# ofsoundof/GRL-Image-Restoration

Hardware: AMD Instinct MI355X
Metric: LQ megapixels/s, GRL-Base x4 SR, 256x256 LQ tiles (higher is better)
Workload: dtype f16 MFMA operands (attention, linear, conv), f32 accumulate + residual stream; 1 GPU; BASELINE configs[2]: GRL-Base x4 SR, 256x256 LQ tiles, ckpt geometry (window 32, stripe 64x64, anchor /2), random-init weights with checkpoint-like logit scales exp(min(ln 100 + 0.3 N(0,1), ln 100)): about half of the heads at the clamp, the regime of every released checkpoint; logit_scale_regime=checkpoint-like, parallelism=tile-sharded x1, no data-path collective, precision_mode=fast

## Files before the change

### grl_image_restoration_amd/csrc/cab_conv2.hip

```cpp
#include "common.h"
#include "grl_hip_internal.h"
#include <stdlib.h>

namespace {

constexpr int C2_TH = 8, C2_TW = 32;
constexpr int C2_HH = C2_TH + 2, C2_HW = C2_TW + 2;
constexpr int C2_SEG = 7;
constexpr int C2_PXB = C2_SEG * 16;
constexpr int C2_NPIECE = C2_HH * C2_HW * C2_SEG;
constexpr int C2_WAVES = 8, C2_THREADS = C2_WAVES * 64;
constexpr int C2_ROUNDS = (C2_NPIECE + C2_THREADS - 1) / C2_THREADS;
constexpr int C2_HALO_B = C2_ROUNDS * C2_THREADS * 16;
constexpr int C2_KSTEPS = 14, C2_NG = 3;
constexpr int C2_KREAL = 9 * 48;

typedef __attribute__((__vector_size__(4 * sizeof(uint32_t)))) uint32_t c2_u32x4;

__global__ __launch_bounds__(C2_THREADS) void cab_conv2_kernel(GrlCabConv2Args p) {
    extern __shared__ __attribute__((aligned(1024))) char smem[];
    const int tid = threadIdx.x, lane = tid & 63, wave = tid >> 6;
    const int wave_u = __builtin_amdgcn_readfirstlane(wave);
    const int r16 = lane & 15, g4 = lane >> 4;
    const int cs = wave_u & 3, ph = wave_u >> 2;
    const int img = blockIdx.x / p.wgs_per_image, wgi = blockIdx.x % p.wgs_per_image;
    const int tiles_x = (p.W + C2_TW - 1) / C2_TW, tiles_y = (p.H + C2_TH - 1) / C2_TH, ntiles = tiles_x * tiles_y;
    const uint32_t lds0 = (uint32_t)(uintptr_t)(__attribute__((address_space(3))) void*)smem;

    gemm_x8 A[C2_NG][C2_KSTEPS];
    {
        const gemm_x8* src = (const gemm_x8*)p.blob + (int64_t)(3 * cs) * C2_KSTEPS * 64 + lane;
#pragma unroll
        for (int g = 0; g < C2_NG; ++g)
#pragma unroll
            for (int s = 0; s < C2_KSTEPS; ++s) A[g][s] = src[(g * C2_KSTEPS + s) * 64];
    }
    f32x4 pool[C2_NG];
#pragma unroll
    for (int g = 0; g < C2_NG; ++g) pool[g] = f32x4{0, 0, 0, 0};
    float* bias_s = (float*)(smem + 2 * C2_HALO_B);
    if (tid < 192) bias_s[tid] = p.bias[tid];
    __syncthreads();
    const float* bias_l = bias_s + 48 * cs + 4 * g4;
    const bool hi2 = g4 >= 2;

    int h0;
    {
        const int px = tid / C2_SEG, seg = tid - px * C2_SEG, hy = px / C2_HW, hx = px - hy * C2_HW;
        h0 = hy << 16 | hx << 4 | seg;
    }
    c2_u32x4 xsrd;
    {
        const uint64_t a = (uint64_t)((const gemm_t*)p.x + (int64_t)img * p.H * p.W * p.ldx);
        xsrd[0] = __builtin_amdgcn_readfirstlane((uint32_t)a);
        xsrd[1] = __builtin_amdgcn_readfirstlane((uint32_t)(a >> 32) & 0xffffu);
        xsrd[2] = (uint32_t)((int64_t)p.H * p.W * p.ldx * 2);
        xsrd[3] = 0x00020000u;
    }
    auto prefetch = [&](int tile, int buf) {
        const int ty = tile / tiles_x, tx = tile - ty * tiles_x;
        const int y0 = ty * C2_TH - 1, x0 = tx * C2_TW - 1;
        int hy = h0 >> 16, hx = (h0 >> 4) & 0xfff, seg = h0 & 15;
#pragma unroll 1
        for (int j = 0; j < C2_ROUNDS; ++j) {
            if (j > 0) {
                static_assert(C2_THREADS == 73 * C2_SEG + 1 && 73 == 2 * C2_HW + 5, "piece stepping");
                seg += 1; hx += 5; hy += 2;
                if (seg >= C2_SEG) { seg -= C2_SEG; hx += 1; }
                if (hx >= C2_HW) { hx -= C2_HW; hy += 1; }
            }
            const int gy = y0 + hy, gx = x0 + hx;
            const bool ok = hy < C2_HH && gy >= 0 && gy < p.H && gx >= 0 && gx < p.W;
            const uint32_t voff = ok ? (uint32_t)(((int64_t)gy * p.W + gx) * p.ldx * 2 + seg * 16) : 0xfffffff0u;
            const uint32_t m0v = __builtin_amdgcn_readfirstlane(lds0 + buf * C2_HALO_B + (j * C2_THREADS + wave_u * 64) * 16);
            asm volatile("s_mov_b32 m0, %0\n\ts_nop 4\n\tbuffer_load_dwordx4 %1, %2, 0 offen lds" ::"s"(m0v), "v"(voff), "s"(xsrd) : "memory");
        }
    };

    int tile = wgi;
    if (tile < ntiles) prefetch(tile, 0);
    for (int it = 0; tile < ntiles; ++it, tile += p.wgs_per_image) {
        asm volatile("s_waitcnt vmcnt(0)" ::: "memory");
        __builtin_amdgcn_s_barrier();
        if (tile + p.wgs_per_image < ntiles) prefetch(tile + p.wgs_per_image, (it + 1) & 1);
        const int ty = tile / tiles_x, tx = tile - ty * tiles_x;
        const char* hb = smem + (it & 1) * C2_HALO_B;
#pragma unroll 1
        for (int rr = 0; rr < 4; ++rr) {
            const int r = 4 * ph + rr;
            const int y = ty * C2_TH + r;
            const char* u0 = hb + (r * C2_HW + r16) * C2_PXB + 16 * g4;
            const char* uA = u0 + (hi2 ? C2_PXB - 96 : 0);
            const char* uB = u0 + (hi2 ? (C2_HW - 2) * C2_PXB - 96 : 0);
            const char* uC = u0 + (hi2 ? -32 : 0);
            f32x4 acc0[C2_NG], acc1[C2_NG];
#pragma unroll
            for (int g = 0; g < C2_NG; ++g) { acc0[g] = *(const f32x4*)(bias_l + 16 * g); acc1[g] = acc0[g]; }
#pragma unroll
            for (int s = 0; s < C2_KSTEPS; ++s) {
                constexpr int TAPOFF[9] = {0, C2_PXB, 2 * C2_PXB, C2_HW * C2_PXB, (C2_HW + 1) * C2_PXB, (C2_HW + 2) * C2_PXB,
// ... 75 lines not shown
```

### grl_image_restoration_amd/csrc/conv.hip

```cpp
#include "common.h"
#include "grl_hip_internal.h"
#include <stdlib.h>

namespace {

constexpr int TH = 8, TW = 32;
constexpr int CWAVES = 8;
constexpr int HALO_W = TW + 2, HALO_H = TH + 2;

template <int KC, int NT>
__global__ __launch_bounds__(CWAVES * 64) void conv3x3_kernel(GrlConvArgs p) {
    extern __shared__ __attribute__((aligned(16))) char smem[];
    constexpr int ROWB = KC * 2 + 16;
    constexpr int KS = KC / 32;
    constexpr int IN_BYTES = HALO_H * HALO_W * ROWB;
    constexpr int WT_BYTES = NT * 16 * ROWB;
    constexpr int SEG_ROW = KC / 8;
    constexpr int WSEGS = NT * 16 * SEG_ROW;
    constexpr int WPT = (WSEGS + CWAVES * 64 - 1) / (CWAVES * 64);
    char* in_s = smem;
    char* wt_s = smem + IN_BYTES;

    const int tid = threadIdx.x, lane = tid & 63, wave = tid >> 6;
    const int r16 = lane & 15, g4 = lane >> 4;
    const int x0 = blockIdx.x * TW, y0 = blockIdx.y * TH, b = blockIdx.z;
    const int nkc = p.CinP / KC;

    f32x4 acc[2][NT];
#pragma unroll
    for (int mt = 0; mt < 2; ++mt)
#pragma unroll
        for (int nt = 0; nt < NT; ++nt) acc[mt][nt] = f32x4{0, 0, 0, 0};

    gemm_x8 wpre[WPT];
    auto load_w = [&](int tap, int kc) {
        const gemm_t* src = (const gemm_t*)p.w + (int64_t)tap * p.w_tap_stride + kc * KC;
#pragma unroll
        for (int i = 0; i < WPT; ++i) {
            const int s = tid + i * CWAVES * 64;
            if (s < WSEGS) {
                const int rr = s / SEG_ROW, cc = s % SEG_ROW;
                wpre[i] = *(const gemm_x8*)(src + (int64_t)rr * p.CinP + cc * 8);
            }
        }
    };
    auto store_w = [&](int buf) {
#pragma unroll
        for (int i = 0; i < WPT; ++i) {
            const int s = tid + i * CWAVES * 64;
            if (s < WSEGS) {
                const int rr = s / SEG_ROW, cc = s % SEG_ROW;
                *(gemm_x8*)(wt_s + buf * WT_BYTES + rr * ROWB + cc * 16) = wpre[i];
            }
        }
    };

    const int csrc = p.x_split == 3 ? p.CinP / 3 : (p.x_split == 2 ? p.CinP / 2 : p.CinP);
    const float xsc = p.x_scale != 0.0f ? p.x_scale : 1.0f;
    const float osc = p.out_scale != 0.0f ? p.out_scale : 1.0f;
    auto stage_input = [&](int kc) {
#pragma unroll 2
        for (int s = tid; s < HALO_H * HALO_W * SEG_ROW; s += CWAVES * 64) {
            const int pix = s / SEG_ROW, cc = s % SEG_ROW;
            const int vch = kc * KC + cc * 8;
            int part = 0, ch0 = vch;
            if (p.x_split >= 2) {
                part = vch / csrc;
                ch0 = vch - part * csrc;
            }
            const int hy = pix / HALO_W, hx = pix % HALO_W;
            const int gy = y0 + hy - 1, gx = x0 + hx - 1;
            gemm_x8 v = {0, 0, 0, 0, 0, 0, 0, 0};
            if (gy >= 0 && gy < p.H && gx >= 0 && gx < p.W) {
                const int64_t row = ((int64_t)b * p.H + gy) * p.W + gx;
                if (p.x_dtype == GRL_DT_F16) {
                    v = *(const gemm_x8*)((const gemm_t*)p.x + row * p.ldx + ch0);
                } else {
                    const float4* q = (const float4*)((const float*)p.x + row * p.ldx + ch0);
                    float4 a0, a1;
                    if (p.x_cols > 0) {
                        a0 = ch0 < p.x_cols ? q[0] : float4{0, 0, 0, 0};
                        a1 = ch0 + 4 < p.x_cols ? q[1] : float4{0, 0, 0, 0};
                    } else {
                        a0 = q[0]; a1 = q[1];
                    }
                    const float e[8] = {a0.x * xsc, a0.y * xsc, a0.z * xsc, a0.w * xsc, a1.x * xsc, a1.y * xsc, a1.z * xsc, a1.w * xsc};
#pragma unroll
                    for (int i = 0; i < 8; ++i) v[i] = to_f16(e[i]);
                    if (p.x_split >= 2 && part == 1) {
#pragma unroll
                        for (int i = 0; i < 8; ++i) v[i] = (f16)(e[i] - (float)v[i]);
                    }
                }
            }
            *(gemm_x8*)(in_s + pix * ROWB + cc * 16) = v;
        }
    };
    auto mfma_tap = [&](int tap, const char* wb) {
        const int dy = tap / 3, dx = tap - dy * 3;
        gemm_x8 af[2][KS];
#pragma unroll
        for (int mt = 0; mt < 2; ++mt)
#pragma unroll
            for (int ks = 0; ks < KS; ++ks)
                af[mt][ks] = *(const gemm_x8*)(in_s + ((wave + dy) * HALO_W + (16 * mt + r16 + dx)) * ROWB + (32 * ks + 8 * g4) * 2);
#pragma unroll
        for (int ks = 0; ks < KS; ++ks) {
#pragma unroll
            for (int nt = 0; nt < NT; ++nt) {
                const gemm_x8 wf = *(const gemm_x8*)(wb + (nt * 16 + r16) * ROWB + (32 * ks + 8 * g4) * 2);
                acc[0][nt] = mfma16_gemm(wf, af[0][ks], acc[0][nt]);
                acc[1][nt] = mfma16_gemm(wf, af[1][ks], acc[1][nt]);
            }
        }
    };

    for (int kc = 0; kc < nkc; ++kc) {
        load_w(0, kc);
        __syncthreads();
        stage_input(kc);
        store_w(0);
        __syncthreads();
        for (int tap = 0; tap < 9; ++tap) {
            if (tap < 8) load_w(tap + 1, kc);
            mfma_tap(tap, wt_s + (tap & 1) * WT_BYTES);
            if (tap < 8) {
                store_w((tap + 1) & 1);
                __syncthreads();
            }
        }
    }

    const int gy = y0 + wave;
    float psum[NT][4];
#pragma unroll
    for (int nt = 0; nt < NT; ++nt)
#pragma unroll
        for (int e = 0; e < 4; ++e) psum[nt][e] = 0.f;

    const bool staged = p.out_dtype != GRL_DT_F32 && p.shuffle_r <= 1 && p.resid == nullptr;
    constexpr int ZSEGS = ((NT * 16 + 31) / 32 * 32 - NT * 16) / 8;
    constexpr int OROW = (NT * 2 + ZSEGS) * 16 + 16;
    if (staged) {
        __syncthreads();
#pragma unroll
        for (int mt = 0; mt < 2; ++mt) {
            const int gx = x0 + 16 * mt + r16;
            const bool valid = gy < p.H && gx < p.W;
            char* prow = smem + (wave * TW + 16 * mt + r16) * OROW;
#pragma unroll
            for (int nt = 0; nt < NT; ++nt) {
                const int c = 16 * nt + 4 * g4;
                const float4 b4 = *(const float4*)(p.bias + c);
                float v[4] = {fmaf(acc[mt][nt][0], osc, b4.x), fmaf(acc[mt][nt][1], osc, b4.y), fmaf(acc[mt][nt][2], osc, b4.z), fmaf(acc[mt][nt][3], osc, b4.w)};
                if (p.act == 1) {
{
                        const f32x2v ga = gelu_erf2(f32x2v{v[0], v[1]}), gb = gelu_erf2(f32x2v{v[2], v[3]});
                        v[0] = ga.x; v[1] = ga.y; v[2] = gb.x; v[3] = gb.y;
                    }
                } else if (p.act == 2) {
#pragma unroll
                    for (int e = 0; e < 4; ++e) v[e] = v[e] > 0.f ? v[e] : v[e] * p.slope;
                }
                if (valid) {
#pragma unroll
                    for (int e = 0; e < 4; ++e) psum[nt][e] += v[e];
                }
                uint2 pk;
                pk.x = pack_f16(v[0], v[1]);
                pk.y = pack_f16(v[2], v[3]);
                *(uint2*)(prow + c * 2) = pk;
            }
        }
        const int zs = (p.ldo >= (NT * 16 + 31) / 32 * 32) ? ZSEGS : 0;
        if (ZSEGS > 0 && tid < TH * TW) {
#pragma unroll
            for (int z = 0; z < ZSEGS; ++z) *(uint4*)(smem + tid * OROW + (NT * 2 + z) * 16) = uint4{0, 0, 0, 0};
        }
        __syncthreads();
        const int SEGS = NT * 2 + zs;
        for (int i = tid; i < TH * TW * SEGS; i += CWAVES * 64) {
            const int px = i / SEGS, sg = i - px * SEGS;
            const int ty = px / TW, tx = px - ty * TW;
            const int oy = y0 + ty, ox = x0 + tx;
            if (oy < p.H && ox < p.W) {
                const int64_t row = ((int64_t)b * p.H + oy) * p.W + ox;
                *(uint4*)((gemm_t*)p.out + row * p.ldo + sg * 8) = *(const uint4*)(smem + px * OROW + sg * 16);
            }
        }
    }
#pragma unroll
    for (int mt = 0; mt < (staged ? 0 : 2); ++mt) {
        const int gx = x0 + 16 * mt + r16;
        const bool valid = gy < p.H && gx < p.W;
        const int64_t row = ((int64_t)b * p.H + gy) * p.W + gx;
#pragma unroll
        for (int nt = 0; nt < NT; ++nt) {
            const int c = 16 * nt + 4 * g4;
            const float4 b4 = *(const float4*)(p.bias + c);
            float v[4] = {fmaf(acc[mt][nt][0], osc, b4.x), fmaf(acc[mt][nt][1], osc, b4.y), fmaf(acc[mt][nt][2], osc, b4.z), fmaf(acc[mt][nt][3], osc, b4.w)};
            if (p.act == 1) {
{
                    const f32x2v ga = gelu_erf2(f32x2v{v[0], v[1]}), gb = gelu_erf2(f32x2v{v[2], v[3]});
                    v[0] = ga.x; v[1] = ga.y; v[2] = gb.x; v[3] = gb.y;
                }
            } else if (p.act == 2) {
#pragma unroll
                for (int e = 0; e < 4; ++e) v[e] = v[e] > 0.f ? v[e] : v[e] * p.slope;
            }
            if (valid) {
                if (p.pool_partial != nullptr) {
#pragma unroll
                    for (int e = 0; e < 4; ++e) psum[nt][e] += v[e];
                }
                if (p.resid != nullptr) {
                    const float4 r4 = *(const float4*)(p.resid + row * p.ldr + c);
                    v[0] += r4.x; v[1] += r4.y; v[2] += r4.z; v[3] += r4.w;
                }
                int64_t orow = row;
                int oc = c;
                bool keep = true;
                if (p.shuffle_r > 1) {
                    const int r = p.shuffle_r, cg = p.shuffle_cg;
                    const int q = c / cg;
                    const int ij = p.shuffle_ij0 + q;
                    oc = c - q * cg;
                    keep = ij < r * r;
                    orow = ((int64_t)b * p.H * r + (gy * r + ij / r)) * (p.W * r) + (gx * r + ij % r);
                }
                if (!keep || (p.n_store > 0 && oc >= p.n_store)) {
                } else if (p.out_dtype != GRL_DT_F32) {
                    uint2 pk;
                    pk.x = pack_f16(v[0], v[1]);
                    pk.y = pack_f16(v[2], v[3]);
                    *(uint2*)((gemm_t*)p.out + orow * p.ldo + oc) = pk;
                } else {
                    *(float4*)((float*)p.out + orow * p.ldo + oc) = float4{v[0], v[1], v[2], v[3]};
                }
            }
        }
    }
    if (p.pool_partial != nullptr) {
        __syncthreads();
        float* red = (float*)smem;
#pragma unroll
        for (int nt = 0; nt < NT; ++nt)
#pragma unroll
            for (int e = 0; e < 4; ++e) {
                const float s = row16_sum(psum[nt][e]);
                if (r16 == 0) red[wave * (NT * 16) + 16 * nt + 4 * g4 + e] = s;
            }
        __syncthreads();
        const int wg = (blockIdx.z * gridDim.y + blockIdx.y) * gridDim.x + blockIdx.x;
        for (int c = tid; c < NT * 16; c += CWAVES * 64) {
            float s = 0.f;
#pragma unroll
            for (int w = 0; w < CWAVES; ++w) s += red[w * (NT * 16) + c];
            p.pool_partial[(int64_t)wg * p.pool_stride + c] = s;
        }
    }
}

template <int KC, int NT>
int launch_conv(const GrlConvArgs& p, hipStream_t st) {
    const dim3 grid((p.W + TW - 1) / TW, (p.H + TH - 1) / TH, p.B);
    const size_t rowb = KC * 2 + 16;
    const size_t lds_in = (size_t)HALO_H * HALO_W * rowb;
    size_t lds = lds_in + 2 * (size_t)NT * 16 * rowb;
    const size_t tile_b = (size_t)TH * TW * (NT * 32 + 32 + 16);
    if (lds < tile_b) lds = tile_b;
    auto kfn = conv3x3_kernel<KC, NT>;
    hipError_t e = hipFuncSetAttribute((const void*)kfn, hipFuncAttributeMaxDynamicSharedMemorySize, (int)lds);
    if (e != hipSuccess) return (int)e;
    hipLaunchKernelGGL(kfn, grid, dim3(CWAVES * 64), lds, st, p);
    GRL_CHECK_LAUNCH();
    return 0;
}

template <int KC>
int launch_conv_nt(const GrlConvArgs& p, hipStream_t st) {
    switch (p.CoutP / 16) {
        case 1: return launch_conv<KC, 1>(p, st);
        case 2: return launch_conv<KC, 2>(p, st);
        case 3: return launch_conv<KC, 3>(p, st);
        case 4: return launch_conv<KC, 4>(p, st);
        case 6: return launch_conv<KC, 6>(p, st);
        case 8: return launch_conv<KC, 8>(p, st);
        case 12: return launch_conv<KC, 12>(p, st);
        default: return GRL_ERR_UNSUPPORTED;
    }
}

__global__ __launch_bounds__(1024) void se_kernel(const float* __restrict__ partial, int wgs_per_image, int CP, int C,
                                                  int Cmid, float inv_hw, const float* __restrict__ w1,
                                                  const float* __restrict__ b1, const float* __restrict__ w2,
                                                  const float* __restrict__ b2, float* __restrict__ scale) {
    __shared__ float part[16][256];
    __shared__ float mean[256];
    __shared__ float mid[64];
    const int b = blockIdx.x, tid = threadIdx.x;
    {
        const int c4 = (tid & 63) * 4, q = tid >> 6;
// ... 25 lines not shown
            for (int o = 32; o >= 1; o >>= 1) s += __shfl_xor(s, o, 64);
            if (lane == 0) mid[j] = fmaxf(s + b1[j], 0.f);
        }
    }
    __syncthreads();
    if (tid < CP) {
        float o = 0.f;
        if (tid < C) {
            float s = b2[tid];
            for (int j = 0; j < Cmid; ++j) s += w2[tid * Cmid + j] * mid[j];
            o = 1.0f / (1.0f + __expf(-s));
        }
        scale[(int64_t)b * CP + tid] = o;
    }
}

}

bool grl_conv192_supported(const GrlConvArgs& p);
int grl_conv192_launch(const GrlConvArgs& p, hipStream_t st);

extern "C" int grl_conv3x3_fwd(void* stream, const GrlConvArgs* args) {
    const GrlConvArgs& p = *args;
    if (p.B <= 0 || p.H <= 0 || p.W <= 0) return GRL_ERR_BAD_ARG;
    if (p.CinP % 32 || p.CoutP % 16 || p.CoutP > 192 || (p.ldx % (p.x_cols > 0 ? 4 : 8)) || (p.ldo % 4)) return GRL_ERR_BAD_ARG;
    if (p.x_cols < 0 || p.n_store < 0) return GRL_ERR_BAD_ARG;
    if (p.x_cols > 0 && ((p.x_cols % 4) || p.x_cols > p.CinP || p.ldx < p.x_cols || p.x_dtype != GRL_DT_F32 || p.x_split >= 2)) return GRL_ERR_BAD_ARG;
    if (p.n_store > 0 && ((p.n_store % 4) || p.n_store > p.CoutP || p.ldo < p.n_store || p.out_dtype != GRL_DT_F32 || p.shuffle_r > 1)) return GRL_ERR_BAD_ARG;
    if (p.x_split < 0 || p.x_split > 3) return GRL_ERR_BAD_ARG;
    if (p.x_split >= 2 && (p.x_dtype != GRL_DT_F32 || p.CinP % (8 * p.x_split) != 0)) return GRL_ERR_BAD_ARG;
    if (p.pool_partial != nullptr && p.pool_stride < p.CoutP) return GRL_ERR_BAD_ARG;
    if (p.shuffle_r > 1 && (p.shuffle_cg <= 0 || (p.shuffle_cg % 4) || (p.CoutP % p.shuffle_cg))) return GRL_ERR_BAD_ARG;
    hipStream_t st = (hipStream_t)stream;
    if (grl_conv192_supported(p)) return grl_conv192_launch(p, st);
    if (p.CinP % 64 == 0) return launch_conv_nt<64>(p, st);
    return launch_conv_nt<32>(p, st);
}

extern "C" int grl_conv3x3_num_workgroups(int32_t B, int32_t H, int32_t W) {
    return B * ((H + TH - 1) / TH) * ((W + TW - 1) / TW);
}

extern "C" int grl_se_scale_fwd(void* stream, const float* pool_partial, int32_t B, int32_t wgs_per_image, int32_t CP,
                                int32_t C, int32_t Cmid, int32_t HW, const float* w1, const float* b1, const float* w2,
                                const float* b2, float* scale) {
    if (CP > 256 || Cmid > 64 || C > CP) return GRL_ERR_BAD_ARG;
    hipLaunchKernelGGL(se_kernel, dim3(B), dim3(1024), 0, (hipStream_t)stream, pool_partial, wgs_per_image, CP, C, Cmid,
                       1.0f / (float)HW, w1, b1, w2, b2, scale);
    GRL_CHECK_LAUNCH();
    return 0;
}
```

### grl_image_restoration_amd/_lib.py

```python
import ctypes as C
import os

from . import switches as SW

_HERE = os.path.dirname(os.path.abspath(__file__))
LIB_PATH = os.path.join(_HERE, "libgrl_hip.so")
ABI_VERSION = 45
DT_F32, DT_BF16, DT_F16 = 0, 1, 2

EPI_PLAIN, EPI_GELU, EPI_GROUPNORM, EPI_LN_RES, EPI_GELU_GRAD = 0, 1, 2, 3, 4

class _Strict(C.Structure):

    def __init__(self, **kw):
        bad = set(kw) - {f[0] for f in self._fields_}
        if bad:
            raise TypeError(f"{type(self).__name__}: unknown field(s) {sorted(bad)}")
        super().__init__(**kw)


class GrlLinearArgs(_Strict):
    _fields_ = [
        ("a", C.c_void_p),
        ("a_dtype", C.c_int32),
        ("lda", C.c_int64),
        ("pool_df", C.c_int32),
        ("pool_H", C.c_int32),
        ("pool_W", C.c_int32),
        ("w", C.c_void_p),
        ("bias", C.c_void_p),
        ("M", C.c_int32),
        ("Npad", C.c_int32),
        ("Kpad", C.c_int32),
        ("epi", C.c_int32),
        ("gscale", C.c_void_p),
        ("ln_g", C.c_void_p),
        ("ln_b", C.c_void_p),
        ("n_real", C.c_int32),
        ("ln_eps", C.c_float),
        ("res_scale", C.c_float),
# ... 165 lines not shown
    ]


class GrlConvArgs(_Strict):
    _fields_ = [
        ("x", C.c_void_p),
        ("x_dtype", C.c_int32),
        ("ldx", C.c_int64),
        ("w", C.c_void_p),
        ("w_tap_stride", C.c_int64),
        ("bias", C.c_void_p),
        ("B", C.c_int32),
        ("H", C.c_int32),
        ("W", C.c_int32),
        ("CinP", C.c_int32),
        ("CoutP", C.c_int32),
        ("x_split", C.c_int32),
        ("x_scale", C.c_float),
        ("out_scale", C.c_float),
        ("act", C.c_int32),
        ("slope", C.c_float),
        ("resid", C.c_void_p),
        ("ldr", C.c_int64),
        ("pool_partial", C.c_void_p),
        ("pool_stride", C.c_int64),
        ("out", C.c_void_p),
        ("out_dtype", C.c_int32),
        ("ldo", C.c_int64),
        ("shuffle_r", C.c_int32),
        ("shuffle_cg", C.c_int32),
        ("shuffle_ij0", C.c_int32),
        ("x_cols", C.c_int32),
        ("n_store", C.c_int32),
    ]


class GrlLnResArgs(_Strict):
    _fields_ = [
        ("x", C.c_void_p),
        ("ldx", C.c_int64),
        ("resid", C.c_void_p),
        ("ldr", C.c_int64),
        ("gamma", C.c_void_p),
        ("beta", C.c_void_p),
        ("add2", C.c_void_p),
        ("add2_dtype", C.c_int32),
        ("ldadd2", C.c_int64),
        ("add2_scale", C.c_void_p),
        ("rows_per_image", C.c_int32),
        ("M", C.c_int32),
        ("n_real", C.c_int32),
        ("n_pad", C.c_int32),
        ("eps", C.c_float),
        ("res_scale", C.c_float),
        ("y", C.c_void_p),
        ("ldy", C.c_int64),
    ]


class GrlGemmTnArgs(_Strict):
    _fields_ = [
        ("a", C.c_void_p),
        ("lda", C.c_int64),
        ("b", C.c_void_p),
        ("b_dtype", C.c_int32),
        ("ldb", C.c_int64),
# ... 710 lines not shown
```

### grl_image_restoration_amd/forward_infer.py

```python
import torch

from . import _lib as L
from . import ops
from . import switches as SW
from .geometry import BlockGeo
from .plan import BlockPlan, Plan


def cab(model, r, pk: BlockPlan, B, H, W, CP):
    hi = pk.hi_c
    sp, dt = (3, torch.float32) if hi else (1, ops.GEMM_DTYPE)
    mid = ops.empty(B * H * W, pk.cab_mid, dtype=dt, device=r.device)
    ops.conv3x3(r, pk.cab0_w, pk.cab0_b, B, H, W, act=1, out=mid, x_split=pk.cab0_split)
    if pk.cab2_blob is not None:
        raw, pool = ops.cab_conv2(mid, pk.cab2_blob, pk.cab2_bias, B, H, W)
    else:
        raw, pool = ops.conv3x3(mid, pk.cab2_w, pk.cab2_b, B, H, W, want_pool=True, out_dtype=dt, x_split=sp)
    gate = ops.se_scale(pool, B, CP, model.embed_dim, H * W, pk.se1_w, pk.se1_b, pk.se3_w, pk.se3_b)
    return raw, gate


def attention(model, qkv, anc, att, pk: BlockPlan, geo: BlockGeo, B, H, W, lse=None, qkv_lo=None, anc_lo=None):
    C = model.embed_dim
    nh_w, nh_s = geo.nh_w, geo.nh_s
# ... 129 lines not shown
    Bg = B // n
    Mg = t.shape[0] // n
    parts = [t[g * Mg : (g + 1) * Mg] for g in range(n)]
    for g in range(n):
        pool[g].wait_stream(main)
    for si, st in enumerate(plan.stages):
        r = list(parts)
        for bi, pk in enumerate(st.blocks):
            for g in range(n):
                with torch.cuda.stream(pool[g]):
                    r[g] = block(model, r[g], pk, plan.sched[si][bi], Bg, H, W)
        for g in range(n):
            with torch.cuda.stream(pool[g]):
                parts[g] = ops.conv3x3(r[g], st.conv_w, st.conv_b, Bg, H, W, resid=parts[g], x_split=plan.xs["stage_conv"])
    out = ops.empty_like(t)
    for g in range(n):
        with torch.cuda.stream(pool[g]):
            ops.layernorm(parts[g], plan.ne_g, plan.ne_b, model.embed_dim, out=out[g * Mg : (g + 1) * Mg])
        main.wait_stream(pool[g])
    return out


def _tokens(x, cpad):
    B, C, H, W = x.shape
    t = torch.zeros(B * H * W, cpad, dtype=torch.float32, device=x.device)
    t[:, :C] = x.permute(0, 2, 3, 1).reshape(-1, C)
    return t


def _image(t, B, H, W, C):
    return t.view(B, H, W, -1)[..., :C].permute(0, 3, 1, 2)


def forward(model, x, plan: Plan):
    B, _, H, W = x.shape
    s, oc = model.upscale, model.out_channels
    sp = plan.split

    def conv(*a, **kw):
        return ops.conv3x3(*a, x_split=sp, **kw)

    bf = torch.float32 if sp == 3 else ops.GEMM_DTYPE

    f = ops.conv3x3(_tokens(x, plan.first[0].shape[2] // 3), *plan.first, B, H, W, x_split=3)
    body = ops.conv3x3(forward_features(model, f, plan, B, H, W), *plan.after, B, H, W, resid=f, x_split=plan.xs["after"])
    if model.upsampler == "pixelshuffle":
        y = conv(body, *plan.cbu, B, H, W, act=2, slope=0.01, out_dtype=bf)
        h, w, r = H, W, plan.ups_r
        for wt, bs in plan.ups:
            y = conv(y, wt, bs, B, h, w, out_dtype=bf, shuffle_r=r, shuffle_cg=64)
            h, w = h * r, w * r
        y = _image(conv(y, *plan.last, B, h, w), B, h, w, oc)
    elif model.upsampler == "pixelshuffledirect":
        y = conv(body, *plan.upd, B, H, W, shuffle_r=s, shuffle_cg=plan.upd_cg)
        y = _image(y, B, H * s, W * s, oc)
    elif model.upsampler == "nearest+conv":
        y = conv(body, *plan.cbu, B, H, W, act=2, slope=0.01, out_dtype=bf)

        def up2(t, h, w):
            return t.view(B, h, 1, w, 1, -1).expand(B, h, 2, w, 2, t.shape[1]).reshape(B * 4 * h * w, -1)

        y = conv(up2(y, H, W), *plan.up1, B, 2 * H, 2 * W, act=2, slope=0.2, out_dtype=bf)
        y = conv(up2(y, 2 * H, 2 * W), *plan.up2, B, 4 * H, 4 * W, act=2, slope=0.2, out_dtype=bf)
        y = conv(y, *plan.hr, B, 4 * H, 4 * W, act=2, slope=0.2, out_dtype=bf)
        y = _image(conv(y, *plan.last, B, 4 * H, 4 * W), B, 4 * H, 4 * W, oc)
    else:
        y = _image(ops.conv3x3(body, *plan.last, B, H, W, x_split=plan.xs["last"]), B, H, W, oc)
        if model.in_channels == model.out_channels:
            y = x + y
    return y
```

### grl_image_restoration_amd/model.py

```python
import math

import torch
import torch.nn as nn
import torch.nn.functional as F

from . import _lib as L
from . import autograd as AG
from . import forward_infer, forward_train, ops
from . import plan as P
from . import switches as SW
from .geometry import pad_multiple, to_2tuple


class _Affine(nn.Module):
    def __init__(self, nh):
        super().__init__()
        self.logit_scale = nn.Parameter(torch.log(10 * torch.ones((nh, 1, 1))))
        self.cpb_mlp = nn.Sequential(nn.Linear(2, 512, bias=True), nn.ReLU(inplace=True), nn.Linear(512, nh, bias=False))


class _Body(nn.Module):
    def __init__(self, body):
        super().__init__()
        self.body = body
# ... 344 lines not shown
        if ent is None:
            with torch.no_grad():
                self._forward_eager(x)
                torch.cuda.synchronize(x.device)
                static_in = x.clone()
                graph = torch.cuda.CUDAGraph()
                with torch.cuda.graph(graph):
                    static_out = self._forward_eager(static_in)
            ent = self._graphs[key] = (static_in, graph, static_out, next(iter(self._plan_cache.values())), stamp)
        static_in, graph, static_out = ent[:3]
        static_in.copy_(x)
        graph.replay()
        return static_out.clone()

    def _forward_eager(self, x, plan=None):
        if not x.is_cuda:
            if SW.on("GRL_NO_CPU_COMPOSITE"):
                raise RuntimeError("grl_image_restoration_amd.GRL: got a CPU tensor and GRL_NO_CPU_COMPOSITE=1 forbids the composite torch path "
                                   "(no CPU fallback)")
            if any(p.is_cuda for p in self.parameters()):
                raise RuntimeError("grl_image_restoration_amd.GRL: CPU input but the parameters live on the GPU")
            from . import composite
            composite.announce()
            return forward_train.forward(self, x)
        L.lib()
        if plan is None and torch.is_grad_enabled() and (x.requires_grad or any(p.requires_grad for p in self.parameters())):
            return forward_train.forward(self, x)
        H0, W0 = x.shape[2:]
        x = self.check_image_size(x.float())
        mean = self._mean.to(x.device, x.dtype)
        x = (x - mean) * self.img_range
        if plan is None:
            plan = self._plan(tuple(x.shape[2:]), x.device)
        y = forward_infer.forward(self, x, plan) / self.img_range + mean
        return y[:, :, : H0 * self.upscale, : W0 * self.upscale].contiguous()
```

### grl_image_restoration_amd/ops.py

```python
import ctypes as C
import os
import dataclasses
from dataclasses import dataclass
from typing import Optional, Tuple

import torch

from . import _lib as L
from . import switches as SW

GEMM_DTYPE = torch.float16
PLANE_DTYPE = torch.float16
_KIND = {torch.float32: L.DT_F32, torch.float16: L.DT_F16}


_POISON = SW.on("GRL_POISON")


GUARD_BYTES = 4096
GUARD_BYTE = 0xA5
_GUARDS = False
_GUARDED: list = []


# ... 601 lines not shown
                     split: int = 1) -> torch.Tensor:
    cout, cin = w.shape[:2]
    w9 = w.detach().float().permute(2, 3, 0, 1).reshape(9, cout, cin)
    out = torch.zeros(9, cout_pad, cin_pad, dtype=torch.float32, device=w.device)
    if shuffle_r > 1:
        r2 = shuffle_r * shuffle_r
        c = cout // r2
        src = w9.view(9, c, r2, cin).permute(0, 2, 1, 3)
        out.view(9, cout_pad // shuffle_cg, shuffle_cg, cin_pad)[:, :r2, :c, :cin] = src
    else:
        out[:, :cout, :cin] = w9
    if split == 3:
        return split3_weight(out)
    if split == 2:
        hi = out.to(GEMM_DTYPE)
        return torch.cat([hi, hi], dim=-1).contiguous()
    return out.to(GEMM_DTYPE).contiguous()


def pack_conv_bias(b: torch.Tensor, cout_pad: int, shuffle_r: int = 0, shuffle_cg: int = 0) -> torch.Tensor:
    out = torch.zeros(cout_pad, dtype=torch.float32, device=b.device)
    if shuffle_r > 1:
        r2 = shuffle_r * shuffle_r
        c = b.numel() // r2
        out.view(cout_pad // shuffle_cg, shuffle_cg)[:r2, :c] = b.detach().float().view(c, r2).t()
    else:
        out[: b.numel()] = b.detach().float()
    return out


def conv3x3(x: torch.Tensor, w: torch.Tensor, bias: torch.Tensor, B: int, H: int, W: int, *, act: int = 0,
            slope: float = 0.0, resid: Optional[torch.Tensor] = None, want_pool: bool = False,
            out_dtype=torch.float32, out: Optional[torch.Tensor] = None, shuffle_r: int = 0, shuffle_cg: int = 0,
            x_split: int = 1, x_scale: float = 1.0, out_scale: float = 1.0, x_cols: int = 0, n_store: int = 0):
    _dev_check(x, w, bias, resid, out)
    assert x.dim() == 2 and x.stride(1) == 1 and x.dtype in (torch.float32, GEMM_DTYPE)
    assert w.dtype == GEMM_DTYPE and w.is_contiguous() and w.dim() == 3 and w.shape[0] == 9
    CoutP, CinP = w.shape[1], w.shape[2]
    assert x_split in (1, 2, 3) and x.shape[0] >= B * H * W and x.shape[1] >= (x_cols if x_cols > 0 else CinP // x_split) and bias.numel() == CoutP
    assert x_split == 1 or x.dtype == torch.float32
    assert x_cols == 0 or (x.dtype == torch.float32 and x_split == 1 and x_cols % 4 == 0 and x.stride(0) % 4 == 0)
    assert n_store == 0 or (n_store % 4 == 0 and n_store <= CoutP and shuffle_r <= 1 and out_dtype == torch.float32 and not want_pool)
    if shuffle_r > 1:
        rows, cols = B * H * W * shuffle_r * shuffle_r, shuffle_cg
    else:
        rows, cols = B * H * W, (n_store if n_store > 0 else CoutP)
    if out is None:
        out = empty(rows, cols, dtype=out_dtype, device=x.device)
    pool = None
    if want_pool:
        nwg = L.lib().grl_conv3x3_num_workgroups(B, H, W)
        pool = empty(nwg, CoutP, dtype=torch.float32, device=x.device)
    step = CoutP
    split = SW.num("GRL_CONV_SPLIT", default=96 if CinP <= 64 and x_split == 1 else 0)
    if split and CoutP > split and CoutP % split == 0 and shuffle_r <= 1:
        step = split
    elif CoutP > 192:
        step = max(s for s in (192, 128, 96, 64, 48, 32, 16) if CoutP % s == 0 and (shuffle_r <= 1 or s % shuffle_cg == 0))
    for c0 in range(0, CoutP, step):
        ns = 0
        if n_store > 0:
            ns = min(step, n_store - c0)
            if ns <= 0:
                continue
            ns = 0 if ns == step else ns
        args = L.GrlConvArgs(
            x=_ptr(x), x_dtype=_KIND[x.dtype], ldx=x.stride(0),
            w=C.c_void_p(w.data_ptr() + c0 * CinP * 2), w_tap_stride=CoutP * CinP,
            bias=C.c_void_p(bias.data_ptr() + c0 * 4),
            B=B, H=H, W=W, CinP=CinP, CoutP=step, x_split=x_split, x_scale=x_scale, out_scale=out_scale, act=act, slope=slope,
            resid=C.c_void_p(resid.data_ptr() + c0 * 4) if resid is not None else C.c_void_p(0),
            ldr=resid.stride(0) if resid is not None else 0,
            pool_partial=C.c_void_p(pool.data_ptr() + c0 * 4) if pool is not None else C.c_void_p(0), pool_stride=CoutP,
            out=C.c_void_p(out.data_ptr() + (0 if shuffle_r > 1 else c0 * out.element_size())),
            out_dtype=_KIND[out.dtype], ldo=out.stride(0),
# ... 672 lines not shown
```

### include/grl_hip.h

```cpp
#ifndef GRL_HIP_H
#define GRL_HIP_H
#include <stdint.h>

#ifdef __cplusplus
extern "C" {
#endif

#define GRL_ERR_BAD_ARG (-1)
#define GRL_ERR_UNSUPPORTED (-2)
#define GRL_ABI_VERSION 45

enum { GRL_DT_F32 = 0, GRL_DT_BF16 = 1, GRL_DT_F16 = 2 };

enum { GRL_EPI_PLAIN = 0, GRL_EPI_GELU = 1, GRL_EPI_GROUPNORM = 2, GRL_EPI_LN_RES = 3,
       GRL_EPI_GELU_GRAD = 4  };

typedef struct GrlLinearArgs {
    const void* a;
    int32_t a_dtype;
    int64_t lda;
    int32_t pool_df;
    int32_t pool_H, pool_W;
    const void* w;
    const float* bias;
    int32_t M, Npad, Kpad;
    int32_t epi;
    const float* gscale;
    const float* ln_g;
    const float* ln_b;
    int32_t n_real;
    float ln_eps;
    float res_scale;
    const float* resid;
    int64_t ldr;
    const void* add2;
    int32_t add2_dtype;
    int64_t ldadd2;
    const float* add2_scale;
    int32_t rows_per_image;
    int32_t a_split;
    float a_scale;
    float out_scale;
    void* out;
// ... 124 lines not shown
    const float* lazy_ceil;
} GrlAttnArgs;

int grl_attention_fwd(void* stream, const GrlAttnArgs* args);

int grl_attention_rows_geometry_ok(const GrlAttnArgs* args);

typedef struct GrlConvArgs {
    const void* x;
    int32_t x_dtype;
    int64_t ldx;
    const void* w;
    int64_t w_tap_stride;
    const float* bias;
    int32_t B, H, W;
    int32_t CinP, CoutP;
    int32_t x_split;
    float x_scale;
    float out_scale;
    int32_t act;
    float slope;
    const float* resid;
    int64_t ldr;
    float* pool_partial;
    int64_t pool_stride;
    void* out;
    int32_t out_dtype;
    int64_t ldo;
    int32_t shuffle_r;
    int32_t shuffle_cg;
    int32_t shuffle_ij0;
    int32_t x_cols;
    int32_t n_store;
} GrlConvArgs;

int grl_conv3x3_fwd(void* stream, const GrlConvArgs* args);
int grl_conv3x3_num_workgroups(int32_t B, int32_t H, int32_t W);

typedef struct GrlCabConv2Args {
    const void* x;
    int64_t ldx;
    const void* blob;
    const float* bias;
    int32_t B, H, W;
    int32_t wgs_per_image;
    void* out;
    int64_t ldo;
    float* pool_partial;
    int64_t pool_stride;
} GrlCabConv2Args;

int grl_cab_conv2_fwd(void* stream, const GrlCabConv2Args* args);
int64_t grl_cab_conv2_blob_bytes(void);

int grl_se_scale_fwd(void* stream, const float* pool_partial, int32_t B, int32_t wgs_per_image, int32_t CP, int32_t C,
                     int32_t Cmid, int32_t HW, const float* w1, const float* b1, const float* w2, const float* b2,
                     float* scale);

int grl_layernorm_fwd(void* stream, const float* x, int64_t ldx, float* y, int64_t ldy, const float* gamma,
                      const float* beta, int32_t M, int32_t n_real, int32_t n_pad, float eps);

typedef struct GrlLnResArgs {
    const float* x;
    int64_t ldx;
    const float* resid;
    int64_t ldr;
// ... 608 lines not shown
```

Baseline: 6.616 LQ megapixels/s.

## Swizzle conv LDS rows instead of padding, stage pixel-shuffle outputs, trim CAB halo segments

The generic 3x3 conv kernel drops the 16-byte row padding in LDS and instead XOR-swizzles the 16-byte segment index per row to avoid bank conflicts. This shrinks the LDS footprint, which may allow more resident workgroups. Pixel-shuffle outputs now also take the LDS-staged, vectorized store path, with the scatter address computed per segment. The CAB conv2 halo uses 6 segments per pixel instead of 7, with the piece-stepping constants updated to match. These changes add index arithmetic, and the reduced segment count only holds if 96 channels per pixel is enough.

```diff
diff --git a/grl_image_restoration_amd/csrc/cab_conv2.hip b/grl_image_restoration_amd/csrc/cab_conv2.hip
--- a/grl_image_restoration_amd/csrc/cab_conv2.hip
+++ b/grl_image_restoration_amd/csrc/cab_conv2.hip
@@ -6,7 +6,7 @@
 
 constexpr int C2_TH = 8, C2_TW = 32;
 constexpr int C2_HH = C2_TH + 2, C2_HW = C2_TW + 2;
-constexpr int C2_SEG = 7;
+constexpr int C2_SEG = 6;
 constexpr int C2_PXB = C2_SEG * 16;
 constexpr int C2_NPIECE = C2_HH * C2_HW * C2_SEG;
 constexpr int C2_WAVES = 8, C2_THREADS = C2_WAVES * 64;
@@ -64,8 +64,8 @@
 #pragma unroll 1
         for (int j = 0; j < C2_ROUNDS; ++j) {
             if (j > 0) {
-                static_assert(C2_THREADS == 73 * C2_SEG + 1 && 73 == 2 * C2_HW + 5, "piece stepping");
-                seg += 1; hx += 5; hy += 2;
+                static_assert(C2_THREADS == 85 * C2_SEG + 2 && 85 == 2 * C2_HW + 17, "piece stepping");
+                seg += 2; hx += 17; hy += 2;
                 if (seg >= C2_SEG) { seg -= C2_SEG; hx += 1; }
                 if (hx >= C2_HW) { hx -= C2_HW; hy += 1; }
             }
diff --git a/grl_image_restoration_amd/csrc/conv.hip b/grl_image_restoration_amd/csrc/conv.hip
--- a/grl_image_restoration_amd/csrc/conv.hip
+++ b/grl_image_restoration_amd/csrc/conv.hip
@@ -11,7 +11,8 @@
 template <int KC, int NT>
 __global__ __launch_bounds__(CWAVES * 64) void conv3x3_kernel(GrlConvArgs p) {
     extern __shared__ __attribute__((aligned(16))) char smem[];
-    constexpr int ROWB = KC * 2 + 16;
+    constexpr int ROWB = KC * 2;
+    auto swz = [](int r) { return KC == 64 ? (r & 7) : ((r >> 1) & 2); };
     constexpr int KS = KC / 32;
     constexpr int IN_BYTES = HALO_H * HALO_W * ROWB;
     constexpr int WT_BYTES = NT * 16 * ROWB;
@@ -50,7 +51,7 @@
             const int s = tid + i * CWAVES * 64;
             if (s < WSEGS) {
                 const int rr = s / SEG_ROW, cc = s % SEG_ROW;
-                *(gemm_x8*)(wt_s + buf * WT_BYTES + rr * ROWB + cc * 16) = wpre[i];
+                *(gemm_x8*)(wt_s + buf * WT_BYTES + rr * ROWB + (cc ^ swz(rr)) * 16) = wpre[i];
             }
         }
     };
@@ -59,7 +60,7 @@
     const float xsc = p.x_scale != 0.0f ? p.x_scale : 1.0f;
     const float osc = p.out_scale != 0.0f ? p.out_scale : 1.0f;
     auto stage_input = [&](int kc) {
-#pragma unroll 2
+#pragma unroll(NT == 1 ? 1 : 2)
         for (int s = tid; s < HALO_H * HALO_W * SEG_ROW; s += CWAVES * 64) {
             const int pix = s / SEG_ROW, cc = s % SEG_ROW;
             const int vch = kc * KC + cc * 8;
@@ -93,22 +94,24 @@
                     }
                 }
             }
-            *(gemm_x8*)(in_s + pix * ROWB + cc * 16) = v;
+            *(gemm_x8*)(in_s + pix * ROWB + (cc ^ swz(pix)) * 16) = v;
         }
     };
     auto mfma_tap = [&](int tap, const char* wb) {
         const int dy = tap / 3, dx = tap - dy * 3;
         gemm_x8 af[2][KS];
 #pragma unroll
-        for (int mt = 0; mt < 2; ++mt)
+        for (int mt = 0; mt < 2; ++mt) {
+            const int row = (wave + dy) * HALO_W + (16 * mt + r16 + dx);
 #pragma unroll
             for (int ks = 0; ks < KS; ++ks)
-                af[mt][ks] = *(const gemm_x8*)(in_s + ((wave + dy) * HALO_W + (16 * mt + r16 + dx)) * ROWB + (32 * ks + 8 * g4) * 2);
+                af[mt][ks] = *(const gemm_x8*)(in_s + row * ROWB + ((4 * ks + g4) ^ swz(row)) * 16);
+        }
 #pragma unroll
         for (int ks = 0; ks < KS; ++ks) {
 #pragma unroll
             for (int nt = 0; nt < NT; ++nt) {
-                const gemm_x8 wf = *(const gemm_x8*)(wb + (nt * 16 + r16) * ROWB + (32 * ks + 8 * g4) * 2);
+                const gemm_x8 wf = *(const gemm_x8*)(wb + (nt * 16 + r16) * ROWB + ((4 * ks + g4) ^ swz(r16)) * 16);
                 acc[0][nt] = mfma16_gemm(wf, af[0][ks], acc[0][nt]);
                 acc[1][nt] = mfma16_gemm(wf, af[1][ks], acc[1][nt]);
             }
@@ -138,7 +141,9 @@
 #pragma unroll
         for (int e = 0; e < 4; ++e) psum[nt][e] = 0.f;
 
-    const bool staged = p.out_dtype != GRL_DT_F32 && p.shuffle_r <= 1 && p.resid == nullptr;
+    const bool shuf = p.shuffle_r > 1;
+    const bool staged = p.out_dtype != GRL_DT_F32 && p.resid == nullptr &&
+                        (!shuf || ((p.shuffle_cg % 8) == 0 && (p.ldo % 8) == 0 && ((uintptr_t)p.out & 15) == 0));
     constexpr int ZSEGS = ((NT * 16 + 31) / 32 * 32 - NT * 16) / 8;
     constexpr int OROW = (NT * 2 + ZSEGS) * 16 + 16;
     if (staged) {
@@ -172,7 +177,7 @@
                 *(uint2*)(prow + c * 2) = pk;
             }
         }
-        const int zs = (p.ldo >= (NT * 16 + 31) / 32 * 32) ? ZSEGS : 0;
+        const int zs = (!shuf && p.ldo >= (NT * 16 + 31) / 32 * 32) ? ZSEGS : 0;
         if (ZSEGS > 0 && tid < TH * TW) {
 #pragma unroll
             for (int z = 0; z < ZSEGS; ++z) *(uint4*)(smem + tid * OROW + (NT * 2 + z) * 16) = uint4{0, 0, 0, 0};
@@ -184,8 +189,17 @@
             const int ty = px / TW, tx = px - ty * TW;
             const int oy = y0 + ty, ox = x0 + tx;
             if (oy < p.H && ox < p.W) {
-                const int64_t row = ((int64_t)b * p.H + oy) * p.W + ox;
-                *(uint4*)((gemm_t*)p.out + row * p.ldo + sg * 8) = *(const uint4*)(smem + px * OROW + sg * 16);
+                int64_t row = ((int64_t)b * p.H + oy) * p.W + ox;
+                int os = sg;
+                bool keep = true;
+                if (shuf) {
+                    const int r = p.shuffle_r, gs = p.shuffle_cg >> 3;
+                    const int q = sg / gs, ij = p.shuffle_ij0 + q;
+                    os = sg - q * gs;
+                    keep = ij < r * r;
+                    row = ((int64_t)b * p.H * r + (oy * r + ij / r)) * (p.W * r) + (ox * r + ij % r);
+                }
+                if (keep) *(uint4*)((gemm_t*)p.out + row * p.ldo + os * 8) = *(const uint4*)(smem + px * OROW + sg * 16);
             }
         }
     }
@@ -264,7 +278,7 @@
 template <int KC, int NT>
 int launch_conv(const GrlConvArgs& p, hipStream_t st) {
     const dim3 grid((p.W + TW - 1) / TW, (p.H + TH - 1) / TH, p.B);
-    const size_t rowb = KC * 2 + 16;
+    const size_t rowb = KC * 2;
     const size_t lds_in = (size_t)HALO_H * HALO_W * rowb;
     size_t lds = lds_in + 2 * (size_t)NT * 16 * rowb;
     const size_t tile_b = (size_t)TH * TW * (NT * 32 + 32 + 16);
```

Result: no change. 6.660 LQ megapixels/s (median of 6 runs) (+0.7%).

## Stage pixel-shuffle conv stores through LDS and fuse final conv into image output

Applied to the files above, without the earlier changes.

Adds an LDS-staged path for pixel-shuffle conv outputs, so the shuffled f16 rows are written as coalesced 16-byte segments instead of scattered per-lane stores. It also fuses the last conv's epilogue with the de-normalisation (divide by img_range, add mean), the NCHW permute and the crop, writing the final image directly. This removes the separate _image permute, the division and addition kernels and the contiguous copy. The cost is extra LDS for the shuffle staging and an uncoalesced NCHW scalar store in the last conv.

```diff
diff --git a/grl_image_restoration_amd/_lib.py b/grl_image_restoration_amd/_lib.py
--- a/grl_image_restoration_amd/_lib.py
+++ b/grl_image_restoration_amd/_lib.py
@@ -5,7 +5,7 @@
 
 _HERE = os.path.dirname(os.path.abspath(__file__))
 LIB_PATH = os.path.join(_HERE, "libgrl_hip.so")
-ABI_VERSION = 45
+ABI_VERSION = 46
 DT_F32, DT_BF16, DT_F16 = 0, 1, 2
 
 EPI_PLAIN, EPI_GELU, EPI_GROUPNORM, EPI_LN_RES, EPI_GELU_GRAD = 0, 1, 2, 3, 4
@@ -237,6 +237,12 @@
         ("shuffle_ij0", C.c_int32),
         ("x_cols", C.c_int32),
         ("n_store", C.c_int32),
+        ("img", C.c_void_p),
+        ("img_C", C.c_int32),
+        ("img_H", C.c_int32),
+        ("img_W", C.c_int32),
+        ("img_mean", C.c_void_p),
+        ("img_range", C.c_float),
     ]
 
 
diff --git a/grl_image_restoration_amd/csrc/conv.hip b/grl_image_restoration_amd/csrc/conv.hip
--- a/grl_image_restoration_amd/csrc/conv.hip
+++ b/grl_image_restoration_amd/csrc/conv.hip
@@ -1,5 +1,6 @@
 #include "common.h"
 #include "grl_hip_internal.h"
+#include <stdint.h>
 #include <stdlib.h>
 
 namespace {
@@ -7,6 +8,11 @@
 constexpr int TH = 8, TW = 32;
 constexpr int CWAVES = 8;
 constexpr int HALO_W = TW + 2, HALO_H = TH + 2;
+
+__host__ __device__ inline bool shuffle_staged(const GrlConvArgs& p) {
+    return p.shuffle_r > 1 && p.out_dtype != GRL_DT_F32 && p.resid == nullptr && p.shuffle_cg >= 32 && p.shuffle_cg % 8 == 0 &&
+           p.ldo % 8 == 0 && ((uintptr_t)p.out & 15) == 0;
+}
 
 template <int KC, int NT>
 __global__ __launch_bounds__(CWAVES * 64) void conv3x3_kernel(GrlConvArgs p) {
@@ -138,7 +144,9 @@
 #pragma unroll
         for (int e = 0; e < 4; ++e) psum[nt][e] = 0.f;
 
-    const bool staged = p.out_dtype != GRL_DT_F32 && p.shuffle_r <= 1 && p.resid == nullptr;
+    const bool staged_sh = shuffle_staged(p);
+    const bool staged = staged_sh || (p.out_dtype != GRL_DT_F32 && p.shuffle_r <= 1 && p.resid == nullptr);
+    const int sh_cg = staged_sh ? p.shuffle_cg : NT * 16, sh_row = sh_cg * 2 + 16;
     constexpr int ZSEGS = ((NT * 16 + 31) / 32 * 32 - NT * 16) / 8;
     constexpr int OROW = (NT * 2 + ZSEGS) * 16 + 16;
     if (staged) {
@@ -151,6 +159,11 @@
 #pragma unroll
             for (int nt = 0; nt < NT; ++nt) {
                 const int c = 16 * nt + 4 * g4;
+                char* dst = prow + c * 2;
+                if (staged_sh) {
+                    const int q = c / sh_cg;
+                    dst = smem + ((q * TH + wave) * TW + 16 * mt + r16) * sh_row + (c - q * sh_cg) * 2;
+                }
                 const float4 b4 = *(const float4*)(p.bias + c);
                 float v[4] = {fmaf(acc[mt][nt][0], osc, b4.x), fmaf(acc[mt][nt][1], osc, b4.y), fmaf(acc[mt][nt][2], osc, b4.z), fmaf(acc[mt][nt][3], osc, b4.w)};
                 if (p.act == 1) {
@@ -169,17 +182,36 @@
                 uint2 pk;
                 pk.x = pack_f16(v[0], v[1]);
                 pk.y = pack_f16(v[2], v[3]);
-                *(uint2*)(prow + c * 2) = pk;
+                *(uint2*)dst = pk;
             }
         }
         const int zs = (p.ldo >= (NT * 16 + 31) / 32 * 32) ? ZSEGS : 0;
-        if (ZSEGS > 0 && tid < TH * TW) {
+        if (ZSEGS > 0 && !staged_sh && tid < TH * TW) {
 #pragma unroll
             for (int z = 0; z < ZSEGS; ++z) *(uint4*)(smem + tid * OROW + (NT * 2 + z) * 16) = uint4{0, 0, 0, 0};
         }
         __syncthreads();
+        if (staged_sh) {
+            const int r = p.shuffle_r, nq = NT * 16 / sh_cg, segc = sh_cg / 8;
+            const int i_lo = p.shuffle_ij0 / r, i_n = (p.shuffle_ij0 + nq - 1) / r - i_lo + 1;
+            for (int idx = tid; idx < i_n * TH * TW * r * segc; idx += CWAVES * 64) {
+                int t = idx / segc;
+                const int sg = idx - t * segc;
+                const int j = t % r;
+                t /= r;
+                const int tx = t % TW;
+                t /= TW;
+                const int ty = t % TH, i = i_lo + t / TH;
+                const int ij = i * r + j, q = ij - p.shuffle_ij0;
+                const int oy = y0 + ty, ox = x0 + tx;
+                if (q >= 0 && q < nq && ij < r * r && oy < p.H && ox < p.W) {
+                    const int64_t orow = ((int64_t)b * p.H * r + (oy * r + i)) * (p.W * r) + (ox * r + j);
+                    *(uint4*)((gemm_t*)p.out + orow * p.ldo + sg * 8) = *(const uint4*)(smem + ((q * TH + ty) * TW + tx) * sh_row + sg * 16);
+                }
+            }
+        }
         const int SEGS = NT * 2 + zs;
-        for (int i = tid; i < TH * TW * SEGS; i += CWAVES * 64) {
+        for (int i = tid; i < (staged_sh ? 0 : TH * TW * SEGS); i += CWAVES * 64) {
             const int px = i / SEGS, sg = i - px * SEGS;
             const int ty = px / TW, tx = px - ty * TW;
             const int oy = y0 + ty, ox = x0 + tx;
@@ -208,7 +240,18 @@
 #pragma unroll
                 for (int e = 0; e < 4; ++e) v[e] = v[e] > 0.f ? v[e] : v[e] * p.slope;
             }
-            if (valid) {
+            if (p.img != nullptr) {
+                if (gy < p.img_H && gx < p.img_W) {
+#pragma unroll
+                    for (int e = 0; e < 4; ++e) {
+                        if (c + e < p.img_C) {
+                            float q = __fmul_rn(v[e], p.img_range);
+                            asm volatile("" : "+v"(q));
+                            p.img[(((int64_t)b * p.img_C + (c + e)) * p.img_H + gy) * p.img_W + gx] = __fadd_rn(q, p.img_mean[c + e]);
+                        }
+                    }
+                }
+            } else if (valid) {
                 if (p.pool_partial != nullptr) {
 #pragma unroll
                     for (int e = 0; e < 4; ++e) psum[nt][e] += v[e];
@@ -267,7 +310,8 @@
     const size_t rowb = KC * 2 + 16;
     const size_t lds_in = (size_t)HALO_H * HALO_W * rowb;
     size_t lds = lds_in + 2 * (size_t)NT * 16 * rowb;
-    const size_t tile_b = (size_t)TH * TW * (NT * 32 + 32 + 16);
+    size_t tile_b = (size_t)TH * TW * (NT * 32 + 32 + 16);
+    if (shuffle_staged(p)) tile_b = (size_t)TH * TW * (NT * 32 + (NT * 16 / p.shuffle_cg) * 16);
     if (lds < tile_b) lds = tile_b;
     auto kfn = conv3x3_kernel<KC, NT>;
     hipError_t e = hipFuncSetAttribute((const void*)kfn, hipFuncAttributeMaxDynamicSharedMemorySize, (int)lds);
@@ -359,6 +403,16 @@
     if (p.pool_partial != nullptr && p.pool_stride < p.CoutP) return GRL_ERR_BAD_ARG;
     if (p.shuffle_r > 1 && (p.shuffle_cg <= 0 || (p.shuffle_cg % 4) || (p.CoutP % p.shuffle_cg))) return GRL_ERR_BAD_ARG;
     hipStream_t st = (hipStream_t)stream;
+    if (p.img != nullptr) {
+        if (p.out_dtype != GRL_DT_F32 || p.shuffle_r > 1 || p.resid != nullptr || p.act != 0 || p.pool_partial != nullptr || p.n_store > 0)
+            return GRL_ERR_BAD_ARG;
+        if (p.img_mean == nullptr || p.img_range == 0.0f || p.img_C <= 0 || p.img_C > p.CoutP || p.img_H <= 0 || p.img_H > p.H ||
+            p.img_W <= 0 || p.img_W > p.W)
+            return GRL_ERR_BAD_ARG;
+        GrlConvArgs q = p;
+        q.img_range = 1.0f / p.img_range;
+        return p.CinP % 64 == 0 ? launch_conv_nt<64>(q, st) : launch_conv_nt<32>(q, st);
+    }
     if (grl_conv192_supported(p)) return grl_conv192_launch(p, st);
     if (p.CinP % 64 == 0) return launch_conv_nt<64>(p, st);
     return launch_conv_nt<32>(p, st);
diff --git a/grl_image_restoration_amd/forward_infer.py b/grl_image_restoration_amd/forward_infer.py
--- a/grl_image_restoration_amd/forward_infer.py
+++ b/grl_image_restoration_amd/forward_infer.py
@@ -185,10 +185,15 @@
     return t.view(B, H, W, -1)[..., :C].permute(0, 3, 1, 2)
 
 
-def forward(model, x, plan: Plan):
+def forward(model, x, plan: Plan, image=None):
     B, _, H, W = x.shape
     s, oc = model.upscale, model.out_channels
     sp = plan.split
+
+    def last(y, h, w):
+        if image is None:
+            return _image(conv(y, *plan.last, B, h, w), B, h, w, oc)
+        return conv(y, *plan.last, B, h, w, image=(oc, image[0], image[1], image[2], model.img_range))
 
     def conv(*a, **kw):
         return ops.conv3x3(*a, x_split=sp, **kw)
@@ -203,7 +208,7 @@
         for wt, bs in plan.ups:
             y = conv(y, wt, bs, B, h, w, out_dtype=bf, shuffle_r=r, shuffle_cg=64)
             h, w = h * r, w * r
-        y = _image(conv(y, *plan.last, B, h, w), B, h, w, oc)
+        y = last(y, h, w)
     elif model.upsampler == "pixelshuffledirect":
         y = conv(body, *plan.upd, B, H, W, shuffle_r=s, shuffle_cg=plan.upd_cg)
         y = _image(y, B, H * s, W * s, oc)
@@ -216,7 +221,7 @@
         y = conv(up2(y, H, W), *plan.up1, B, 2 * H, 2 * W, act=2, slope=0.2, out_dtype=bf)
         y = conv(up2(y, 2 * H, 2 * W), *plan.up2, B, 4 * H, 4 * W, act=2, slope=0.2, out_dtype=bf)
         y = conv(y, *plan.hr, B, 4 * H, 4 * W, act=2, slope=0.2, out_dtype=bf)
-        y = _image(conv(y, *plan.last, B, 4 * H, 4 * W), B, 4 * H, 4 * W, oc)
+        y = last(y, 4 * H, 4 * W)
     else:
         y = _image(ops.conv3x3(body, *plan.last, B, H, W, x_split=plan.xs["last"]), B, H, W, oc)
         if model.in_channels == model.out_channels:
diff --git a/grl_image_restoration_amd/model.py b/grl_image_restoration_amd/model.py
--- a/grl_image_restoration_amd/model.py
+++ b/grl_image_restoration_amd/model.py
@@ -400,5 +400,8 @@
         x = (x - mean) * self.img_range
         if plan is None:
             plan = self._plan(tuple(x.shape[2:]), x.device)
+        if self.upsampler in ("pixelshuffle", "nearest+conv") and mean.numel() in (1, self.out_channels):
+            mvec = mean.reshape(-1).expand(self.out_channels).contiguous()
+            return forward_infer.forward(self, x, plan, image=(H0 * self.upscale, W0 * self.upscale, mvec))
         y = forward_infer.forward(self, x, plan) / self.img_range + mean
         return y[:, :, : H0 * self.upscale, : W0 * self.upscale].contiguous()
diff --git a/grl_image_restoration_amd/ops.py b/grl_image_restoration_amd/ops.py
--- a/grl_image_restoration_amd/ops.py
+++ b/grl_image_restoration_amd/ops.py
@@ -657,7 +657,8 @@
 def conv3x3(x: torch.Tensor, w: torch.Tensor, bias: torch.Tensor, B: int, H: int, W: int, *, act: int = 0,
             slope: float = 0.0, resid: Optional[torch.Tensor] = None, want_pool: bool = False,
             out_dtype=torch.float32, out: Optional[torch.Tensor] = None, shuffle_r: int = 0, shuffle_cg: int = 0,
-            x_split: int = 1, x_scale: float = 1.0, out_scale: float = 1.0, x_cols: int = 0, n_store: int = 0):
+            x_split: int = 1, x_scale: float = 1.0, out_scale: float = 1.0, x_cols: int = 0, n_store: int = 0,
+            image: Optional[tuple] = None):
     _dev_check(x, w, bias, resid, out)
     assert x.dim() == 2 and x.stride(1) == 1 and x.dtype in (torch.float32, GEMM_DTYPE)
     assert w.dtype == GEMM_DTYPE and w.is_contiguous() and w.dim() == 3 and w.shape[0] == 9
@@ -666,6 +667,23 @@
     assert x_split == 1 or x.dtype == torch.float32
     assert x_cols == 0 or (x.dtype == torch.float32 and x_split == 1 and x_cols % 4 == 0 and x.stride(0) % 4 == 0)
     assert n_store == 0 or (n_store % 4 == 0 and n_store <= CoutP and shuffle_r <= 1 and out_dtype == torch.float32 and not want_pool)
+    if image is not None:
+        iC, iH, iW, imean, irange = image
+        assert out_dtype == torch.float32 and act == 0 and resid is None and shuffle_r <= 1 and not want_pool and n_store == 0
+        assert CoutP <= 192 and 0 < iC <= CoutP and 0 < iH <= H and 0 < iW <= W and float(irange) != 0.0
+        assert imean.dtype == torch.float32 and imean.is_contiguous() and imean.numel() == iC and imean.device == x.device
+        img = out if out is not None else empty(B, iC, iH, iW, dtype=torch.float32, device=x.device)
+        assert img.shape == (B, iC, iH, iW) and img.dtype == torch.float32 and img.is_contiguous()
+        args = L.GrlConvArgs(
+            x=_ptr(x), x_dtype=_KIND[x.dtype], ldx=x.stride(0), w=_ptr(w), w_tap_stride=CoutP * CinP, bias=_ptr(bias),
+            B=B, H=H, W=W, CinP=CinP, CoutP=CoutP, x_split=x_split, x_scale=x_scale, out_scale=out_scale, act=0, slope=0.0,
+            resid=C.c_void_p(0), ldr=0, pool_partial=C.c_void_p(0), pool_stride=CoutP, out=C.c_void_p(0), out_dtype=L.DT_F32, ldo=CoutP,
+            shuffle_r=0, shuffle_cg=0, shuffle_ij0=0, x_cols=x_cols, n_store=0,
+            img=_ptr(img), img_C=iC, img_H=iH, img_W=iW, img_mean=_ptr(imean), img_range=float(irange),
+        )
+        with _timed(f"conv3x3 {CinP}->{CoutP} {H}x{W} image" if _PROFILE is not None else "conv3x3"):
+            L.launch("grl_conv3x3_fwd", args)
+        return img
     if shuffle_r > 1:
         rows, cols = B * H * W * shuffle_r * shuffle_r, shuffle_cg
     else:
diff --git a/include/grl_hip.h b/include/grl_hip.h
--- a/include/grl_hip.h
+++ b/include/grl_hip.h
@@ -8,7 +8,7 @@
 
 #define GRL_ERR_BAD_ARG (-1)
 #define GRL_ERR_UNSUPPORTED (-2)
-#define GRL_ABI_VERSION 45
+#define GRL_ABI_VERSION 46
 
 enum { GRL_DT_F32 = 0, GRL_DT_BF16 = 1, GRL_DT_F16 = 2 };
 
@@ -199,6 +199,11 @@
     int32_t shuffle_ij0;
     int32_t x_cols;
     int32_t n_store;
+    float* img;
+    int32_t img_C;
+    int32_t img_H, img_W;
+    const float* img_mean;
+    float img_range;
 } GrlConvArgs;
 
 int grl_conv3x3_fwd(void* stream, const GrlConvArgs* args);
```

Result: no change. 6.566 LQ megapixels/s before, 6.565 LQ megapixels/s after, median of 2 (-0.0%).
